# EthanD11/RS-VIO

Hardware: AMD Instinct MI355X
Metric: stereo frames/sec (tracker+BA) on 752×480 EuRoC stream; BA ms/iter at window=10 (higher is better)
Workload: dtype f32 (tracker) / f64 (BA)

## Files before the change

### rs-vio_amd/csrc/ba.hip

```cpp
#include <rccl/rccl.h>

#include <algorithm>
#include <chrono>
#include <cmath>
#include <cstdlib>
#include <cstring>
#include <string>
#include <sys/resource.h>
#include <numeric>
#include <stdexcept>
#include <vector>

#include "common.hpp"

#include "obs_pass.hpp"
#include "se3.hpp"
#include "wave.hpp"

#pragma clang fp contract(fast)

namespace rsvio {

namespace {

// ... 297 lines not shown
    const int i = blockIdx.x * blockDim.x + threadIdx.x;
    if (i < 7 * G.n_kf) {
        Wk.pose[0][i] = Wk.pose_init[i];
        Wk.pose[1][i] = Wk.pose_init[i];
    }
    if (i < 3 * G.n_lm) {
        Wk.pw[0][i] = Wk.pw_init[i];
        Wk.pw[1][i] = Wk.pw_init[i];
    }
    if (i == 0) {
        Wk.tick[1] = wall_clock64();
        *Wk.singular = 0;
        LmState s{};
        s.lambda = lambda0;
        s.nu = 2.0;
        *Wk.st = s;
    }
}

struct SlotLin {
    double V[6], gp[3], Wr[9], Ur[6], gr[3], cost;
};

__device__ __forceinline__ void slot_linearize(const Geometry& G, const Pose& P, const double p[3], int nobs,
                                               int cams, const double2 (&uvq)[2], bool fr, SlotLin& L) {
#pragma unroll
    for (int i = 0; i < 6; ++i) L.V[i] = 0.0;
#pragma unroll
    for (int i = 0; i < 3; ++i) L.gp[i] = 0.0;
#pragma unroll
    for (int i = 0; i < 9; ++i) L.Wr[i] = 0.0;
#pragma unroll
    for (int i = 0; i < 6; ++i) L.Ur[i] = 0.0;
#pragma unroll
    for (int i = 0; i < 3; ++i) L.gr[i] = 0.0;
    L.cost = 0.0;
#pragma unroll
    for (int o = 0; o < 2; ++o) {
        if (o >= nobs) break;
        double r[2], J[2][9];
        const double uv[2] = {uvq[o].x, uvq[o].y};
        linearize(p, P, G.TCB[(cams >> o) & 1].m, uv, r, J, true);
        double sq = r[0] * r[0] + r[1] * r[1], rho, wt;
        huber(sq, G.huber_delta, &rho, &wt);
        L.cost += 0.5 * rho;
        const double wr0 = wt * r[0], wr1 = wt * r[1];
        int k = 0;
#pragma unroll
        for (int a = 0; a < 3; ++a) {
#pragma unroll
            for (int c = a; c < 3; ++c) L.V[k++] += wt * (J[0][a] * J[0][c] + J[1][a] * J[1][c]);
            L.gp[a] += J[0][a] * wr0 + J[1][a] * wr1;
        }
        if (fr) {
            int u = 0;
#pragma unroll
            for (int a = 0; a < 3; ++a) {
#pragma unroll
                for (int c = 0; c < 3; ++c) L.Wr[a * 3 + c] += wt * (J[0][6 + a] * J[0][c] + J[1][6 + a] * J[1][c]);
#pragma unroll
                for (int c = a; c < 3; ++c) L.Ur[u++] += wt * (J[0][6 + a] * J[0][6 + c] + J[1][6 + a] * J[1][6 + c]);
                L.gr[a] += J[0][6 + a] * wr0 + J[1][6 + a] * wr1;
            }
        }
    }
}

__device__ __forceinline__ void wave_sync() {
// ... 2305 lines not shown
        if (i < n) {
            Wk.dc[i] = x[q];
            dcs[i] = x[q];
        }
    }
    __builtin_amdgcn_s_waitcnt(0xc07f);
    __builtin_amdgcn_wave_barrier();
    if (lane < G.n_kf) {
        double* qd = Wk.pose[1 - st->cur] + 7 * lane;
        if (fidx < 0) {
#pragma unroll
            for (int i = 0; i < 7; ++i) qd[i] = p7[i];
        } else {
            double qv[7];
            se3_plus(p7, dcs + 6 * fidx, qv);
#pragma unroll
            for (int i = 0; i < 7; ++i) qd[i] = qv[i];
        }
    }
    if (lane == 0) k5_result(st, 1, d2, gd);
    STAMP(5);
}

template <bool FUSED>
__device__ void k6_body(const Geometry& G, const Prob& Pr, const Work& Wk, int w, int lane, double (*sh)[64],
                        double (*shp)[64], double (*shs)[64], const P2P* PP = nullptr,
                        unsigned long long gen = 0, unsigned long long* k6tag = nullptr,
                        unsigned long long* k6part = nullptr) {
    const int s = 64 * w + lane;
    const int4 h0 = Pr.slot_hdr[2 * s], h1 = Pr.slot_hdr[2 * s + 1];
    const double2 uvq[2] = {Pr.slot_uv[2 * s], Pr.slot_uv[2 * s + 1]};
    const LmState* st = Wk.st;
    const bool act = h1.y > 0;
    const int kf = h0.x, l = h0.y, first = act ? h0.z : lane, nk = act ? h0.w : 1;
    const bool fr = h1.x >= 0;
    const int kfc = act ? kf : 0, lc = act ? l : 0, fc = (act && fr) ? h1.x : 0;
    double recb[2][18], Lmb[2][10], pcb[2][3], p7b[2][7], d6[6];
#pragma unroll
    for (int b = 0; b < 2; ++b) {
        const double2* wr = reinterpret_cast<const double2*>(Wk.raws[b] + (size_t)s * kRawF);
#pragma unroll
        for (int i = 0; i < 9; ++i) {
            const double2 x = wr[i];
            recb[b][2 * i] = x.x; recb[b][2 * i + 1] = x.y;
        }
        const double2* lr = reinterpret_cast<const double2*>(Wk.rawl[b] + (size_t)lc * kLmF);
#pragma unroll
        for (int i = 0; i < 5; ++i) {
            const double2 x = lr[i];
            Lmb[b][2 * i] = x.x; Lmb[b][2 * i + 1] = x.y;
        }
#pragma unroll
        for (int i = 0; i < 3; ++i) pcb[b][i] = Wk.pw[b][3 * lc + i];
#pragma unroll
        for (int i = 0; i < 7; ++i) p7b[b][i] = Wk.pose[b][7 * kfc + i];
    }
#pragma unroll
    for (int i = 0; i < 6; ++i) d6[i] = Wk.dc[6 * fc + i];
    const int done = st->done, solve_ok = st->solve_ok, cur = st->cur;
    const double lambda = st->lambda;
#pragma unroll
    for (int b = 0; b < 2; ++b) {
#pragma unroll
        for (int i = 0; i < 18; ++i) __asm__ volatile("" ::"v"(recb[b][i]));
#pragma unroll
        for (int i = 0; i < 10; ++i) __asm__ volatile("" ::"v"(Lmb[b][i]));
#pragma unroll
        for (int i = 0; i < 3; ++i) __asm__ volatile("" ::"v"(pcb[b][i]));
#pragma unroll
        for (int i = 0; i < 7; ++i) __asm__ volatile("" ::"v"(p7b[b][i]));
    }
    if (done || !solve_ok) return;
    STAMP(20);
    RTSTAMP(7);
    double Wv[18], Lm[10], pc[3], p7[7];
    {
        double rec[18];
#pragma unroll
        for (int i = 0; i < 18; ++i) rec[i] = cur ? recb[1][i] : recb[0][i];
        slot_w(rec, Wv);
#pragma unroll
        for (int i = 0; i < 10; ++i) Lm[i] = cur ? Lmb[1][i] : Lmb[0][i];
#pragma unroll
        for (int i = 0; i < 3; ++i) pc[i] = cur ? pcb[1][i] : pcb[0][i];
#pragma unroll
        for (int i = 0; i < 7; ++i) p7[i] = cur ? p7b[0][i] : p7b[1][i];
    }
    double t3[3] = {0.0, 0.0, 0.0};
    if (act && fr) {
#pragma unroll
        for (int c = 0; c < 3; ++c) {
            double acc = 0.0;
#pragma unroll
// ... 17 lines not shown
        double* pt = Wk.pw[1 - cur] + 3 * l;
        double dp2 = 0.0, gpdp = 0.0, p2 = 0.0;
#pragma unroll
        for (int c = 0; c < 3; ++c) {
            const double dp = (Vi[c][0] * rhs[0] + Vi[c][1] * rhs[1]) + Vi[c][2] * rhs[2];
            const double p = pc[c];
            const double q = p + dp;
            shp[c][lane] = q;
            pt[c] = q;
            dp2 += dp * dp;
            gpdp += Lm[LG + c] * dp;
            p2 += p * p;
        }
        shs[1][lane] = dp2;
        shs[2][lane] = gpdp;
        shs[3][lane] = p2;
    }
    if constexpr (FUSED) wave_sync(); else __syncthreads();
    STAMP(23);
    SlotLin L;
    if (act) {
        const Pose P = pose_from7(p7);
        const double q[3] = {shp[0][first], shp[1][first], shp[2][first]};
        slot_linearize(G, P, q, h1.y, h1.z, uvq, fr, L);
    } else {
        const Pose P{};
        const double q[3] = {0.0, 0.0, 1.0};
        slot_linearize(G, P, q, 0, 0, uvq, false, L);
    }
    shs[0][lane] = L.cost;
    if constexpr (FUSED) wave_sync(); else __syncthreads();
    STAMP(24);
    store_linearization<FUSED>(Wk, 1 - cur, s, lane, act, fr, first, nk, l, L, sh);
    STAMP(25);
    {
        double v[kPartD];
#pragma unroll
        for (int i = 0; i < kPartD; ++i) v[i] = wave_sum_det(shs[i][lane]);
        if (lane == 0)
#pragma unroll
            for (int i = 0; i < kPartD; ++i) Wk.partD[w * kPartD + i] = v[i];
        if (k6tag && lane < kPartD) {
            double vl = v[0];
#pragma unroll
            for (int i = 1; i < kPartD; ++i) vl = lane == i ? v[i] : vl;
            const unsigned long long b = (unsigned long long)__double_as_longlong(vl), t = gen << 32;
            const size_t nw = (size_t)G.n_wave;
            __hip_atomic_store(k6tag + (2 * lane) * nw + w, (b & 0xffffffffull) | t, __ATOMIC_RELAXED,
                               __HIP_MEMORY_SCOPE_AGENT);
            __hip_atomic_store(k6tag + (2 * lane + 1) * nw + w, (b >> 32) | t, __ATOMIC_RELAXED,
                               __HIP_MEMORY_SCOPE_AGENT);
        }
        if (k6part && lane < kPartD) {
            double vl = v[0];
#pragma unroll
            for (int i = 1; i < kPartD; ++i) vl = lane == i ? v[i] : vl;
            __hip_atomic_store(k6part + (size_t)w * kPartD + lane, (unsigned long long)__double_as_longlong(vl),
                               __ATOMIC_RELAXED, __HIP_MEMORY_SCOPE_AGENT);
        }
        if (PP && lane < PP->nranks) {
            const int par = (int)(gen & 1);
            double* q = p2p_tval(PP->peer[lane], par, PP->rank, w);
            q[0] = v[0]; q[1] = v[1]; q[2] = v[2]; q[3] = v[3];
            __threadfence_system();
            __hip_atomic_store(p2p_tflag(PP->peer[lane], par, PP->rank, w), gen, __ATOMIC_RELEASE,
                               __HIP_MEMORY_SCOPE_SYSTEM);
        }
    }
    STAMP(21);
    RTSTAMP(8);
}

__global__ __launch_bounds__(64) void ba_backsub_relinearize(Geometry G, Prob Pr, Work Wk) {
    __shared__ double sh[10][64];
    __shared__ double shp[3][64];
    __shared__ double shs[4][64];
    RTSTAMP(6);
    k6_body<false>(G, Pr, Wk, blockIdx.x, threadIdx.x, sh, shp, shs);
    RTSTAMP(9);
}

__global__ __launch_bounds__(64) void ba_backsub_relinearize_p2p(Geometry G, Prob Pr, Work Wk, P2P P,
                                                                 const unsigned long long* xgen) {
    __shared__ double sh[10][64];
    __shared__ double shp[3][64];
    __shared__ double shs[4][64];
    unsigned long long gen = *xgen;
    __asm__ volatile("" : "+s"(gen));
    k6_body<false>(G, Pr, Wk, blockIdx.x, threadIdx.x, sh, shp, shs, &P, gen);
}

template <int KU>
__device__ void k6_reduce_p2p(const Geometry& G, const Prob& Pr, const Work& Wk, const P2P& P,
                              unsigned long long* xgen, int* err, const unsigned long long* k6tag) {
    const int lane = threadIdx.x & 63;
    const LmState s = *Wk.st;
    const unsigned long long gen = *xgen + 1;
    if (s.done) return;
    const unsigned g32 = (unsigned)gen;
    const int nr = P.nranks, me = P.rank, par = (int)(gen & 1);
    const int el = 7 * G.n_kf - 1;
    double p0[3], p1[3];
// ... 200 lines not shown
    }
}

__global__ __launch_bounds__(64) void ba_reduce_trial(Geometry G, Prob Pr, Work Wk, int include_poses) {
    const LmState s = *Wk.st;
    if (s.done) return;
    double v[4];
    trial_scalars_wave(G, Pr, Wk, s, include_poses, v);
    if (threadIdx.x == 0)
        for (int k = 0; k < 4; ++k) Wk.trial4[k] = v[k];
}

constexpr int kK7Threads = 256;
#ifndef RSVIO_K7_BLOCKS
#define RSVIO_K7_BLOCKS 16
#endif
constexpr int kK7Blocks = RSVIO_K7_BLOCKS;
__device__ __forceinline__ void lm_decide_body(const Geometry& G, const Prob& Pr, const Work& Wk, int pre_reduced,
                                               const LmArgs& la, LmState* host, unsigned long long* htick,
                                               double* hout, const P2P* PP = nullptr,
                                               const unsigned long long* xgen = nullptr, int* err = nullptr) {
    STAMP(8);
    __shared__ LmState sd;
    if (threadIdx.x < 64) {
        const LmState d = lm_decide(G, Pr, Wk, Wk.st_prev, pre_reduced, la, PP, xgen, err);
        if (threadIdx.x == 0) {
            sd = d;
            if (blockIdx.x == 0) {
                LmState h = d;
                h.p2p_err = Wk.p2p_err ? *Wk.p2p_err : 0;
                *Wk.st = d;
                *host = h;
            }
        }
    }
    __syncthreads();
    const LmState s = sd;
    if (hout && s.done) {
        const double* pose = Wk.pose[s.cur];
        const double* pw = Wk.pw[s.cur];
        const int np = 7 * G.n_kf, n = np + 3 * G.n_lm;
        const int per = (((n + (int)gridDim.x - 1) / (int)gridDim.x) + 1) & ~1;
        const int i0 = (int)blockIdx.x * per, i1 = min(n, i0 + per);
        for (int i = i0 + 2 * (int)threadIdx.x; i < i1; i += 2 * kK7Threads) {
            const double a = i < np ? pose[i] : pw[i - np];
            if (i + 1 < i1) {
                const double b = i + 1 < np ? pose[i + 1] : pw[i + 1 - np];
                *reinterpret_cast<double2*>(hout + i) = make_double2(a, b);
            } else {
                hout[i] = a;
            }
        }
        __threadfence_system();
        __syncthreads();
        if (threadIdx.x == 0)
            __hip_atomic_store(htick + 4 + blockIdx.x, Wk.tick[1], __ATOMIC_RELEASE, __HIP_MEMORY_SCOPE_SYSTEM);
    }
    if (blockIdx.x == 0 && threadIdx.x == 0) {
        const unsigned long long t = Wk.tick[0] + 1;
        Wk.tick[0] = t;
        htick[1] = Wk.tick[1];
        htick[2] = wall_clock64();
        __threadfence_system();
        __hip_atomic_store(htick, t, __ATOMIC_RELEASE, __HIP_MEMORY_SCOPE_SYSTEM);
    }
    STAMP(10);
}

__global__ __launch_bounds__(kK7Threads) void ba_lm_decide(Geometry G, Prob Pr, Work Wk, int pre_reduced, LmArgs la,
                                                           LmState* host, unsigned long long* htick, double* hout) {
    lm_decide_body(G, Pr, Wk, pre_reduced, la, host, htick, hout);
}

__global__ __launch_bounds__(kK7Threads) void ba_lm_decide_p2p(Geometry G, Prob Pr, Work Wk, LmArgs la, LmState* host,
                                                               unsigned long long* htick, double* hout, P2P P,
                                                               const unsigned long long* xgen, int* err, int mode) {
    lm_decide_body(G, Pr, Wk, mode, la, host, htick, hout, &P, xgen, err);
}

// ... 46 lines not shown
template <int NF>
__global__ __launch_bounds__(64 * kBkWaves) void bab_camera_solve_blk(const WinDesc* __restrict__ D, int wi) {
    const WinDesc& d = D[blockIdx.x];
    const int skip = d.skip;
    const Prob Pr = d.Pr;
    const Work& Wk = d.W[wi];
    desc_touch(Pr.free_idx, Pr.dmap, Wk.pose[0], Wk.pose[1], Wk.cpart, Wk.partA, Wk.singular, Wk.st);
    if (skip) return;
    camera_solve_blk_body<NF>(d.G, Pr, Wk, 1);
}

__global__ __launch_bounds__(64) void bab_backsub_relinearize(const WinDesc* __restrict__ D, int wi) {
    const WinDesc& d = D[blockIdx.y];
    const int skip = d.skip, bound = d.G.n_wave;
    const Prob Pr = d.Pr;
    const Work& Wk = d.W[wi];
    desc_touch(Pr.slot_hdr, Pr.slot_uv, Wk.st, Wk.raws[0], Wk.raws[1], Wk.rawl[0], Wk.rawl[1], Wk.pw[0], Wk.pw[1],
               Wk.pose[0], Wk.pose[1], Wk.dc);
    if (skip | ((int)blockIdx.x >= bound)) return;
    __shared__ double sh[10][64];
    __shared__ double shp[3][64];
    __shared__ double shs[4][64];
    k6_body<false>(d.G, Pr, Wk, blockIdx.x, threadIdx.x, sh, shp, shs);
}

__global__ __launch_bounds__(kK7Threads) void bad_lm_decide(const WinDesc* __restrict__ D, int wi, LmArgs la,
                                                            LmState* host, unsigned long long* htick, double* hout) {
    const WinDesc& d = D[0];
    const Prob Pr = d.Pr;
    const Work& Wk = d.W[wi];
    lm_decide_body(d.G, Pr, Wk, 0, la, host, htick, hout);
}

__global__ __launch_bounds__(64) void bab_lm_decide(const WinDesc* __restrict__ D, int wi, LmArgs la, LmState* host) {
    const WinDesc& d = D[blockIdx.x];
    if (d.skip) return;
    const LmState s = lm_decide(d.G, d.Pr, d.W[wi], d.W[wi].st, 0, la);
    if (threadIdx.x == 0) {
        *d.W[wi].st = s;
        host[blockIdx.x] = s;
    }
}


__device__ void p2p_exchange(const double* msg, int n, const P2P& P, unsigned long long* xgen, int* err, double* out,
                             unsigned long long gen_pre = 0) {
// ... 238 lines not shown
        const bool topo = sl.exec && k_ok && same_cfg(sl.cfg, cfg) && sl.exp == export_on && sl.nf == G.n_free &&
                          sl.coll == coll;
        const bool hit = topo && (dm ? (sl.dptr == dptr() && sl.chunk == G.n_chunk && G.n_wave <= sl.wcap &&
                                        2 * G.n_wave > sl.wcap)
                                     : !sl.stale);
        if (hit) k = sl.k;
        if (!hit) {
            const auto tg0 = std::chrono::steady_clock::now();
            bool try_update = topo && sl.k == k && graph_update;
            if (try_update && hipEventQuery(sl.ev_launch) != hipSuccess) {
                (void)hipGetLastError();
                try_update = false;
            }
            if (!try_update) drop_slot(sl);
            if (hipStreamBeginCapture(stream, hipStreamCaptureModeThreadLocal) != hipSuccess) {
                (void)hipGetLastError();
                graphs_ok = false;
                return false;
            }
            bool ok = true;
            try {
                if (dm) {
                    enqueue_start_d(cfg.lambda_init, wcap);
                    for (int i = 0; i < k; ++i) enqueue_iteration_d(cfg, i, wcap);
                    enqueue_decide_d(cfg, k);
                } else {
                    enqueue_start(cfg.lambda_init);
                    for (int i = 0; i < k; ++i) enqueue_iteration(cfg, i);
                    enqueue_decide(cfg, k);
                }
            } catch (...) {
                ok = false;
            }
            hipGraph_t g = nullptr;
            if (hipStreamEndCapture(stream, &g) != hipSuccess) ok = false;
            const auto tg1 = std::chrono::steady_clock::now();
            bool updated = false;
            if (ok && try_update) {
                hipGraphNode_t err_node = nullptr;
                hipGraphExecUpdateResult r = hipGraphExecUpdateError;
                updated = hipGraphExecUpdate(sl.exec, g, &err_node, &r) == hipSuccess && r == hipGraphExecUpdateSuccess;
                if (!updated) {
                    (void)hipGetLastError();
                    drop_slot(sl);
                }
            }
            if (ok && !updated && hipGraphInstantiate(&sl.exec, g, nullptr, nullptr, 0) != hipSuccess) {
                sl.exec = nullptr;
                ok = false;
            }
            const auto tg2 = std::chrono::steady_clock::now();
// ... 25 lines not shown
        return true;
    }
    int last_iterations = 3;
    DevBuf<double> d_pose2, d_pw2;
    DevBuf<uint8_t> d_arena;
    HostBuf<uint8_t> h_arena;
    bool up_pending = false;
    struct ArenaLayout {
        size_t desc, pose_init, pw_init, free_idx, pb_fa, pb_fb, dmap, mask, lm_base, wave_fill, wave_lm, key, ouv, upload;
        size_t hdr, uv, pairs, total;
    } lay{};
    bool prof_env = false;
    bool prof_slow = false;
    std::string prof_maps;
    bool uv_env = true;
    bool early_env = false;
    bool stage_kernel = true;
    bool stage_split = true;
    const void* h_arena_dev = nullptr;
    HostBuf<double> h_out;
    bool state_export = false, export_on = false;
    bool state_fresh = false;
    std::vector<int> hs_free, hs_pb_fa, hs_pb_fb;
    DevBuf<double> d_raws, d_rawl, d_partA, d_partD, d_cpart, d_sys, d_dc, d_trial4;
    DevBuf<int> d_singular;
    size_t n_pad = 0;
    DevBuf<LmState> d_state;
    HostBuf<LmState> h_state;
    DevBuf<unsigned long long> d_tick;
    unsigned long long* h_tick = nullptr;
    unsigned long long n_tick = 0;
    bool settled = true, tick_wait = true;
    double wclk_khz = 1.0e5;
    ncclComm_t comm = nullptr;
    int nranks = 1, rank = 0;
    int coll = 0;
    bool sharded() const { return coll != 0; }
    double* xbuf = nullptr;
    P2P p2p{};
    bool p2p_opened[kP2PMax] = {};
    DevBuf<int> d_p2p_err;
    DevBuf<unsigned long long> d_xgen;
    DevBuf<int> d_xnw;
    DevBuf<unsigned long long> d_k6tag;
    DevBuf<unsigned> d_k6cnt;

    void init(const rsvio_ba_params& p) {
        P = p;
        if (P.max_keyframes < 2 || P.max_keyframes > kMaxFree + 1 || P.max_landmarks < 1 ||
            P.max_landmarks > (1 << 26) || P.max_observations < 1)
            throw std::invalid_argument("invalid BA capacities (max_keyframes in [2, 21], max_landmarks <= 2^26)");
        RSVIO_HIP(hipSetDevice(P.device));
        RSVIO_HIP(hipStreamCreateWithFlags(&stream, hipStreamNonBlocking));
        RSVIO_HIP(hipEventCreate(&ev0));
        RSVIO_HIP(hipEventCreate(&ev1));
        RSVIO_HIP(hipEventCreateWithFlags(&gv.ev_launch, hipEventDisableTiming));
        RSVIO_HIP(hipEventCreateWithFlags(&gd.ev_launch, hipEventDisableTiming));
        RSVIO_HIP(hipEventCreateWithFlags(&ev_desc, hipEventDisableTiming));
        const char* fv = std::getenv("RSVIO_P2P_FOLD");
        if (fv && fv[0] >= '0' && fv[0] <= '4') fold_lvl = fold_req = fv[0] - '0';
        const char* dv = std::getenv("RSVIO_BA_DESC");
        desc_on = !(dv && dv[0] == '0');
        const char* gu = std::getenv("RSVIO_BA_GRAPH_UPDATE");
        graph_update = !(gu && gu[0] == '0');
        h_state.alloc(1, hipHostMallocCoherent);
        h_out.alloc((size_t)7 * P.max_keyframes + (size_t)3 * P.max_landmarks, hipHostMallocCoherent);
        d_tick.alloc(2);
        RSVIO_HIP(hipMemset(d_tick.p, 0, 2 * sizeof(unsigned long long)));
        RSVIO_HIP(hipHostMalloc(reinterpret_cast<void**>(&h_tick), (4 + kK7Blocks) * sizeof(unsigned long long),
                                hipHostMallocCoherent));
        std::memset(h_tick, 0, (4 + kK7Blocks) * sizeof(unsigned long long));
        {
            int khz = 0;
            if (hipDeviceGetAttribute(&khz, hipDeviceAttributeWallClockRate, P.device) == hipSuccess && khz > 0)
                wclk_khz = khz;
        }
        const char* wv = std::getenv("RSVIO_BA_WAIT");
        tick_wait = !(wv && std::strcmp(wv, "sync") == 0);
        const char* ge = std::getenv("RSVIO_BA_GRAPHS");
        graphs_ok = !(ge && ge[0] == '0');
        const char* pv = std::getenv("RSVIO_BA_PROFILE");
        prof_env = pv != nullptr;
        prof_slow = pv && std::strcmp(pv, "slow") == 0;
        const char* u32v = std::getenv("RSVIO_BA_UV32");
        uv_env = !(u32v && u32v[0] == '0');
        const char* ecv = std::getenv("RSVIO_BA_EARLY_COPY");
        early_env = ecv && ecv[0] == '1';
        const char* stv = std::getenv("RSVIO_BA_STAGE");
        stage_kernel = !(stv && std::strcmp(stv, "sdma") == 0);
        if (stage_kernel) early_env = false;
        const char* ssv = std::getenv("RSVIO_BA_STAGE_SPLIT");
// ... 100 lines not shown
        int ntm = 0;
        auto faults = [] {
            struct rusage ru;
            getrusage(RUSAGE_THREAD, &ru);
            return (long)ru.ru_minflt;
        };
        long f0 = prof ? faults() : 0;
        auto mark = [&] {
            if (!prof) return;
            const auto t = std::chrono::steady_clock::now();
            const long f = faults();
            tms[ntm] = std::chrono::duration<double, std::micro>(t - tp0).count();
            flt[ntm++] = f - f0;
            tp0 = t;
            f0 = f;
        };
        if (pend.active) throw CallOrderError("set_problem: a solve is in flight (call rsvio_ba_wait first)");
        if (graph_update && gv.exec)
            gv.stale = true;
        else
            drop_slot(gv);
        solves_of_problem = 0;
        state_export = false;
        if (n_kf < 1 || n_kf > P.max_keyframes || n_lm < 0 || n_lm > P.max_landmarks || n_obs < 0 ||
            n_obs > P.max_observations)
            throw std::invalid_argument("problem exceeds the handle's capacities");
        auto& free_idx = hs_free;
        free_idx.assign(n_kf, -1);
        int n_free = 0;
        for (int k = 0; k < n_kf; ++k)
            if (!kf_fixed[k]) free_idx[k] = n_free++;
        if (n_free > kMaxFree) throw std::invalid_argument("too many free keyframes");
        if (n_free < 1) throw std::invalid_argument("no free keyframe");
        auto &pb_fa = hs_pb_fa, &pb_fb = hs_pb_fb;
        pb_fa.clear();
        pb_fb.clear();
        for (int a = 0; a < n_free; ++a)
            for (int b = a; b < n_free; ++b) {
                pb_fa.push_back(a);
                pb_fb.push_back(b);
            }
        const int n_pb = (int)pb_fa.size();
        const int n_chunk = kGrp * n_pb;
        auto al = [](size_t b) { return (b + 255) & ~(size_t)255; };
        const size_t nl1 = (size_t)std::max(n_lm, 1);
        ArenaLayout L{};
        size_t off = 0;
        L.desc = off;      off += al(sizeof(WinDesc));
        L.pose_init = off; off += al(sizeof(double) * 7 * (size_t)n_kf);
        L.pw_init = off;   off += al(sizeof(double) * 3 * nl1);
        L.free_idx = off;  off += al(sizeof(int) * (size_t)n_kf);
        L.pb_fa = off;     off += al(sizeof(int) * (size_t)n_pb);
        L.pb_fb = off;     off += al(sizeof(int) * (size_t)n_pb);
        L.dmap = off;      off += al(sizeof(int) * ((size_t)36 * n_pb + 12 * n_free));
        L.lm_base = off;   off += al(sizeof(int) * nl1);
        L.wave_fill = off; off += al(sizeof(int) * nl1);
        L.wave_lm = off;   off += al(sizeof(int) * (nl1 + 1));
        L.mask = off;      off += al(sizeof(unsigned long long) * nl1);
        L.key = off;       off += al(sizeof(unsigned) * std::max(n_obs, 1));
        L.ouv = off;       off += al(sizeof(double2) * std::max(n_obs, 1));
        L.upload = off;
        mark();
        if (up_pending) settle();
        if (h_arena.n < L.upload) {
            h_arena.alloc(L.upload + L.upload / 4, hipHostMallocCoherent);
            void* dp = nullptr;
            RSVIO_HIP(hipHostGetDevicePointer(&dp, h_arena.p, 0));
            h_arena_dev = dp;
        }
        uint8_t* hb = h_arena.p;
        mark();
        auto* m2 = reinterpret_cast<unsigned long long*>(hb + L.mask);
        auto* key = reinterpret_cast<unsigned*>(hb + L.key);
        bool uv32 = false;
        if (!observation_pass(n_obs, obs_lm, obs_kf, obs_cam, obs_uv, n_lm, n_kf, key, m2,
                              uv_env ? reinterpret_cast<float*>(hb + L.ouv) : nullptr, &uv32)) {
            std::memset(m2, 0, sizeof(unsigned long long) * (size_t)n_lm);
            int cl = -1;
            unsigned long long cm = 0;
            for (int i = 0; i < n_obs; ++i) {
                const int l = obs_lm[i], k = obs_kf[i], c = obs_cam[i];
                if (l < 0 || l >= n_lm || k < 0 || k >= n_kf || c > 1)
                    throw std::invalid_argument("observation index out of range");
                if (l != cl) {
                    if (cl >= 0) m2[cl] = cm;
                    cl = l;
                    cm = m2[l];
                }
// ... 61 lines not shown
        if (n_wave) wave_fill[n_wave - 1] = fill;
        wave_lm[n_wave] = n_lm;
        int stride = 1;
        for (int x = 0; x < kGrp; ++x) stride = std::max(stride, gl[x]);
        n_pad = (size_t)64 * n_wave;
        if (coll == 2 && fold_lvl == 2 && n_wave > kP2PWaves)
            throw std::invalid_argument("shard exceeds the folded P2P trial exchange (16384 waves): RSVIO_P2P_FOLD=1");
        mark();
        L.hdr = off;   off += al(sizeof(int4) * 2 * std::max<size_t>(n_pad, 1));
        L.uv = off;    off += al(sizeof(double2) * 2 * std::max<size_t>(n_pad, 1));
        L.pairs = off; off += al(sizeof(int4) * (size_t)n_chunk * stride);
        L.total = off;
        if (d_arena.n < L.total) {
            d_arena.alloc(L.total + L.total / 4);
            if (stage_split) stage(L.mask, L.upload);
            if (early_env)
                RSVIO_HIP(hipMemcpyAsync(d_arena.p + L.mask, hb + L.mask, L.upload - L.mask, hipMemcpyHostToDevice,
                                         stream));
        }
        lay = L;
        std::memcpy(hb + L.pose_init, pose7, sizeof(double) * 7 * (size_t)n_kf);
        if (n_lm) std::memcpy(hb + L.pw_init, pW, sizeof(double) * 3 * (size_t)n_lm);
        std::memcpy(hb + L.free_idx, free_idx.data(), sizeof(int) * (size_t)n_kf);
        std::memcpy(hb + L.pb_fa, pb_fa.data(), sizeof(int) * (size_t)n_pb);
        std::memcpy(hb + L.pb_fb, pb_fb.data(), sizeof(int) * (size_t)n_pb);
        if (n_free <= 10)
            mf_dense_map(n_free, n_pb, pb_fa.data(), pb_fb.data(), reinterpret_cast<int*>(hb + L.dmap));
        else
            mf_dense_map(n_free, n_pb, pb_fa.data(), pb_fb.data(), reinterpret_cast<int*>(hb + L.dmap),
                         6 * bk_template_nf(n_free), kBkLd);
        G.n_kf = n_kf; G.n_free = n_free; G.n_lm = n_lm; G.n_obs = n_obs; G.n_slot = (int)n_pad;
        G.n_pb = n_pb; G.n_wave = n_wave; G.n_chunk = n_chunk; G.pair_stride = stride;
        for (int k = 0, run = -1; k < kMaxFree; ++k) {
            run = std::max(run, cand[k]);
            G.env[k] = (unsigned char)(k >= n_free ? k : want_env ? std::max(k, run) : n_free - 1);
        }
        G.env_on = want_env ? 1 : 0;
        for (int c = 0; c < 2; ++c)
            for (int i = 0; i < 16; ++i) G.TCB[c].m[i] = TCB2[16 * c + i];
        grow_buffers();
        fill_desc(hdesc);
        std::memcpy(hb + L.desc, &hdesc, sizeof(WinDesc));
        mark();
        if (stage_kernel) {
            stage(0, stage_split ? L.mask : L.upload);
        } else {
            RSVIO_HIP(hipMemcpyAsync(d_arena.p, hb, early_env ? L.mask : L.upload, hipMemcpyHostToDevice, stream));
        }
        up_pending = true;
        {
            SlotSrc S;
            S.mask = reinterpret_cast<const unsigned long long*>(d_arena.p + L.mask);
            S.lm_base = reinterpret_cast<const int*>(d_arena.p + L.lm_base);
// ... 132 lines not shown
                if (k5_variant == 2) {
                    const dim3 b3(64 * kBkWaves);
                    switch (bk_template_nf(G.n_free)) {
                        case 13: hipLaunchKernelGGL(ba_camera_solve_blk<13>, g, b3, 0, stream, G, pr, wk, combine); break;
                        case 16: hipLaunchKernelGGL(ba_camera_solve_blk<16>, g, b3, 0, stream, G, pr, wk, combine); break;
                        default: hipLaunchKernelGGL(ba_camera_solve_blk<20>, g, b3, 0, stream, G, pr, wk, combine); break;
                    }
                    break;
                }
                const dim3 b2(64 * kX2Waves);
                if (G.n_free <= 13) hipLaunchKernelGGL(ba_camera_solve_x2<13>, g, b2, 0, stream, G, pr, wk, combine);
                else if (G.n_free <= 16) hipLaunchKernelGGL(ba_camera_solve_x2<16>, g, b2, 0, stream, G, pr, wk, combine);
                else hipLaunchKernelGGL(ba_camera_solve_x2<20>, g, b2, 0, stream, G, pr, wk, combine);
                break;
            }
        }
        RSVIO_HIP(hipGetLastError());
    }

    static LmArgs lm_args(const rsvio_lm_cfg& cfg) {
        return LmArgs{cfg.max_iterations, cfg.cost_tolerance, cfg.parameter_tolerance};
    }

    void enqueue_iteration(const rsvio_lm_cfg& cfg, int it) {
        const Prob pr = prob();
        const Work wk = work(it);
        if (p2p_fold()) {
            if (p2p_fold2() || p2p_fold4())
                hipLaunchKernelGGL(ba_schur_chunks_p2p, dim3(G.n_chunk), dim3(kSchurThreads), 0, stream, G, pr, wk,
                                   lm_args(cfg), p2p, d_xgen.p, d_p2p_err.p, p2p_fold4() ? 4 : 2);
            else
                hipLaunchKernelGGL(ba_schur_chunks, dim3(G.n_chunk), dim3(kSchurThreads), 0, stream, G, pr, wk,
                                   lm_args(cfg), 1);
            RSVIO_HIP(hipGetLastError());
            switch (G.n_free) {
#define RSVIO_CAMP(NF) \
    case NF:                                                                                                            \
        if (p2p.ll)                                                                                                     \
            hipLaunchKernelGGL((ba_camera_solve_mfma_p2p<NF, true>), dim3(1), dim3(kK5Threads), 0, stream, G, pr, wk,  \
                               p2p, d_xgen.p, d_p2p_err.p);                                                            \
        else                                                                                                            \
            hipLaunchKernelGGL((ba_camera_solve_mfma_p2p<NF, false>), dim3(1), dim3(kK5Threads), 0, stream, G, pr, wk, \
                               p2p, d_xgen.p, d_p2p_err.p);                                                            \
        break;
                RSVIO_CAMP(1) RSVIO_CAMP(2) RSVIO_CAMP(3) RSVIO_CAMP(4) RSVIO_CAMP(5)
                RSVIO_CAMP(6) RSVIO_CAMP(7) RSVIO_CAMP(8) RSVIO_CAMP(9) RSVIO_CAMP(10)
#undef RSVIO_CAMP
// ... 3 lines not shown
        } else {
            enqueue_linear_system(it, lm_args(cfg), false);
            launch_camera_solve(pr, wk, sharded() ? 0 : 1);
        }
        if (p2p_fold2()) {
            if (G.n_wave)
                hipLaunchKernelGGL(ba_backsub_relinearize_p2p, dim3(G.n_wave), dim3(64), 0, stream, G, pr, wk, p2p,
                                   d_xgen.p);
            RSVIO_HIP(hipGetLastError());
            return;
        }
        if (p2p_fold4()) {
            hipLaunchKernelGGL(ba_backsub_relinearize_p2p4, dim3(std::max(G.n_wave, 1)), dim3(64), 0, stream, G, pr,
                               wk, p2p, d_xgen.p, d_k6cnt.p, d_k6tag.p);
            RSVIO_HIP(hipGetLastError());
            return;
        }
        if (p2p_fold3()) {
            hipLaunchKernelGGL(ba_backsub_relinearize_p2p3, dim3(G.n_wave + 1), dim3(64), 0, stream, G, pr, wk, p2p,
                               d_xgen.p, d_p2p_err.p, d_k6tag.p);
            RSVIO_HIP(hipGetLastError());
            return;
        }
        if (G.n_wave) hipLaunchKernelGGL(ba_backsub_relinearize, dim3(G.n_wave), dim3(64), 0, stream, G, pr, wk);
        RSVIO_HIP(hipGetLastError());
        if (coll == 2) {
            hipLaunchKernelGGL(ba_p2p_trial, dim3(1), dim3(256), 0, stream, G, pr, wk, p2p, d_xgen.p, d_p2p_err.p);
            RSVIO_HIP(hipGetLastError());
        } else if (sharded()) {
            hipLaunchKernelGGL(ba_reduce_trial, dim3(1), dim3(64), 0, stream, G, pr, wk, rank == 0 ? 1 : 0);
            RSVIO_HIP(hipGetLastError());
            allreduce(d_trial4.p, 4);
        }
    }

    void enqueue_decide(const rsvio_lm_cfg& cfg, int it) {
        if (p2p_fold2() || p2p_fold4()) {
            hipLaunchKernelGGL(ba_lm_decide_p2p, dim3(export_on ? kK7Blocks : 1), dim3(kK7Threads), 0, stream, G,
                               prob(), work(it), lm_args(cfg), h_state.p, h_tick, export_on ? h_out.p : nullptr, p2p,
                               d_xgen.p, d_p2p_err.p, p2p_fold4() ? 4 : 2);
            RSVIO_HIP(hipGetLastError());
            return;
        }
        hipLaunchKernelGGL(ba_lm_decide, dim3(export_on ? kK7Blocks : 1), dim3(kK7Threads), 0, stream, G, prob(),
                           work(it), sharded() ? 1 : 0, lm_args(cfg), h_state.p, h_tick, export_on ? h_out.p : nullptr);
        RSVIO_HIP(hipGetLastError());
    }

    void enqueue_start_d(double lambda0, int wcap) {
        hipLaunchKernelGGL(bab_linearize, dim3(wcap, 1), dim3(64), 0, stream, dptr(), lambda0);
        RSVIO_HIP(hipGetLastError());
    }
    void enqueue_iteration_d(const rsvio_lm_cfg& cfg, int it, int wcap) {
        const int wi = it & 1;
        hipLaunchKernelGGL(bab_schur_chunks, dim3(G.n_chunk, 1), dim3(kSchurThreads), 0, stream, dptr(), wi, lm_args(cfg));
        RSVIO_HIP(hipGetLastError());
        switch (G.n_free) {
#define RSVIO_CAMD(NF) \
    case NF: hipLaunchKernelGGL(bab_camera_solve<NF>, dim3(1), dim3(kK5Threads), 0, stream, dptr(), wi); break;
            RSVIO_CAMD(1) RSVIO_CAMD(2) RSVIO_CAMD(3) RSVIO_CAMD(4) RSVIO_CAMD(5)
            RSVIO_CAMD(6) RSVIO_CAMD(7) RSVIO_CAMD(8) RSVIO_CAMD(9) RSVIO_CAMD(10)
#undef RSVIO_CAMD
            default: throw std::logic_error("descriptor mode: more than 10 free keyframes");
        }
        RSVIO_HIP(hipGetLastError());
        hipLaunchKernelGGL(bab_backsub_relinearize, dim3(wcap, 1), dim3(64), 0, stream, dptr(), wi);
        RSVIO_HIP(hipGetLastError());
    }
    void enqueue_decide_d(const rsvio_lm_cfg& cfg, int it) {
        hipLaunchKernelGGL(bad_lm_decide, dim3(export_on ? kK7Blocks : 1), dim3(kK7Threads), 0, stream, dptr(), it & 1,
                           lm_args(cfg), h_state.p, h_tick, export_on ? h_out.p : nullptr);
        RSVIO_HIP(hipGetLastError());
    }

    struct Pending {
        bool active = false, skipped = false;
        bool by_tick = false;
        rsvio_lm_cfg cfg{};
        int enq = 0, max_it = 0;
    } pend;

    void enqueue_chunk(int k) {
        settled = false;
        for (int i = 0; i < k; ++i) enqueue_iteration(pend.cfg, pend.enq + i);
        pend.enq += k;
        enqueue_decide(pend.cfg, pend.enq);
        ++n_tick;
        if (!pend.by_tick) RSVIO_HIP(hipEventRecord(ev1, stream));
    }

    void resync_ticks() noexcept {
        (void)hipStreamSynchronize(stream);
        (void)hipGetLastError();
        settled = true;
        unsigned long long t = 0;
        if (hipMemcpy(&t, d_tick.p, sizeof t, hipMemcpyDeviceToHost) == hipSuccess) n_tick = t;
        pend.active = false;
    }

    void start(const rsvio_lm_cfg& cfg) {
        if (!has_problem) throw std::invalid_argument("no problem uploaded");
        if (pend.active) throw CallOrderError("a solve is already in flight (call finish first)");
        try {
            start_impl(cfg);
        } catch (...) {
            resync_ticks();
            throw;
        }
    }

    void start_impl(const rsvio_lm_cfg& cfg) {
        G.huber_delta = cfg.huber_delta;
        G.chol = cfg.linear_solver == RSVIO_SOLVER_CHOLESKY ? 1 : 0;
        pend = Pending{};
        pend.active = true;
        pend.cfg = cfg;
        pend.by_tick = by_tick();
        state_export = false;
        if (!sharded() && (G.n_obs < 6 || G.n_obs < G.n_kf + G.n_lm)) {
            pend.skipped = true;
            return;
        }
        pend.max_it = std::max(cfg.max_iterations, 1);
        settled = false;
        state_fresh = false;
        if (!pend.by_tick) RSVIO_HIP(hipEventRecord(ev0, stream));
        int k = std::min(std::max(last_iterations, 1), pend.max_it);
        if (start_graph(cfg, k)) {
            ++n_tick;
            pend.enq += k;
            if (!pend.by_tick) RSVIO_HIP(hipEventRecord(ev1, stream));
        } else {
            enqueue_start(cfg.lambda_init);
            enqueue_chunk(k);
        }
    }

    void finish(rsvio_ba_result* res) {
        if (!pend.active) throw CallOrderError("no solve in flight");
        try {
            finish_impl(res);
        } catch (...) {
            resync_ticks();
            throw;
        }
    }

    void finish_impl(rsvio_ba_result* res) {
        pend.active = false;
        res->iterations = 0;
        if (pend.skipped) {
            res->status = RSVIO_LM_SKIPPED;
            res->initial_cost = res->final_cost = 0.0;
// ... 712 lines not shown
```

Baseline: 4892.

## Fuse final-iteration state export into cost-only backsub kernel and cache host tables

On the last iteration of a chunk, a new backsub kernel variant computes only the trial cost, skipping Jacobian and linearization stores. It also writes the current pose and landmark state into the host output buffer and stamps tick slots so lm_decide can skip its own export copy. If more iterations are then needed, the full relinearization is re-enqueued before the next chunk. Separately, the upload path skips rebuilding the pair and dense-map tables when a key of arena base, offsets, keyframe count and fixed mask is unchanged, which adds cache-validity risk.

```diff
diff --git a/rs-vio_amd/csrc/ba.hip b/rs-vio_amd/csrc/ba.hip
--- a/rs-vio_amd/csrc/ba.hip
+++ b/rs-vio_amd/csrc/ba.hip
@@ -343,28 +343,32 @@
     double V[6], gp[3], Wr[9], Ur[6], gr[3], cost;
 };
 
+template <bool COST_ONLY = false>
 __device__ __forceinline__ void slot_linearize(const Geometry& G, const Pose& P, const double p[3], int nobs,
                                                int cams, const double2 (&uvq)[2], bool fr, SlotLin& L) {
-#pragma unroll
-    for (int i = 0; i < 6; ++i) L.V[i] = 0.0;
-#pragma unroll
-    for (int i = 0; i < 3; ++i) L.gp[i] = 0.0;
-#pragma unroll
-    for (int i = 0; i < 9; ++i) L.Wr[i] = 0.0;
-#pragma unroll
-    for (int i = 0; i < 6; ++i) L.Ur[i] = 0.0;
-#pragma unroll
-    for (int i = 0; i < 3; ++i) L.gr[i] = 0.0;
+    if constexpr (!COST_ONLY) {
+#pragma unroll
+        for (int i = 0; i < 6; ++i) L.V[i] = 0.0;
+#pragma unroll
+        for (int i = 0; i < 3; ++i) L.gp[i] = 0.0;
+#pragma unroll
+        for (int i = 0; i < 9; ++i) L.Wr[i] = 0.0;
+#pragma unroll
+        for (int i = 0; i < 6; ++i) L.Ur[i] = 0.0;
+#pragma unroll
+        for (int i = 0; i < 3; ++i) L.gr[i] = 0.0;
+    }
     L.cost = 0.0;
 #pragma unroll
     for (int o = 0; o < 2; ++o) {
         if (o >= nobs) break;
         double r[2], J[2][9];
         const double uv[2] = {uvq[o].x, uvq[o].y};
-        linearize(p, P, G.TCB[(cams >> o) & 1].m, uv, r, J, true);
+        linearize(p, P, G.TCB[(cams >> o) & 1].m, uv, r, J, !COST_ONLY);
         double sq = r[0] * r[0] + r[1] * r[1], rho, wt;
         huber(sq, G.huber_delta, &rho, &wt);
         L.cost += 0.5 * rho;
+        if constexpr (COST_ONLY) continue;
         const double wr0 = wt * r[0], wr1 = wt * r[1];
         int k = 0;
 #pragma unroll
@@ -2716,11 +2720,21 @@
     STAMP(5);
 }
 
-template <bool FUSED>
+#ifndef RSVIO_EXPORT_FENCE
+#define RSVIO_EXPORT_FENCE 0
+#endif
+__device__ __forceinline__ void export_done() {
+#if RSVIO_EXPORT_FENCE
+    __builtin_amdgcn_fence(__ATOMIC_RELEASE, "");
+#else
+    __builtin_amdgcn_s_waitcnt(kWaitStores);
+#endif
+}
+template <bool FUSED, bool LAST = false>
 __device__ void k6_body(const Geometry& G, const Prob& Pr, const Work& Wk, int w, int lane, double (*sh)[64],
                         double (*shp)[64], double (*shs)[64], const P2P* PP = nullptr,
                         unsigned long long gen = 0, unsigned long long* k6tag = nullptr,
-                        unsigned long long* k6part = nullptr) {
+                        unsigned long long* k6part = nullptr, double* hout = nullptr) {
     const int s = 64 * w + lane;
     const int4 h0 = Pr.slot_hdr[2 * s], h1 = Pr.slot_hdr[2 * s + 1];
     const double2 uvq[2] = {Pr.slot_uv[2 * s], Pr.slot_uv[2 * s + 1]};
@@ -2751,6 +2765,18 @@
     }
 #pragma unroll
     for (int i = 0; i < 6; ++i) d6[i] = Wk.dc[6 * fc + i];
+    const int xnp = 7 * G.n_kf, xn = xnp + 3 * G.n_lm;
+    const int xi = (int)min(2ll * s, (long long)xn);
+    double xv[2][2] = {{0.0, 0.0}, {0.0, 0.0}};
+    unsigned long long xstamp = 0;
+    if constexpr (LAST) {
+#pragma unroll
+        for (int b = 0; b < 2; ++b)
+#pragma unroll
+            for (int e = 0; e < 2; ++e)
+                if (xi + e < xn) xv[b][e] = xi + e < xnp ? Wk.pose[b][xi + e] : Wk.pw[b][xi + e - xnp];
+        xstamp = Wk.tick[1];
+    }
     const int done = st->done, solve_ok = st->solve_ok, cur = st->cur;
     const double lambda = st->lambda;
 #pragma unroll
@@ -2763,6 +2789,34 @@
         for (int i = 0; i < 3; ++i) __asm__ volatile("" ::"v"(pcb[b][i]));
 #pragma unroll
         for (int i = 0; i < 7; ++i) __asm__ volatile("" ::"v"(p7b[b][i]));
+    }
+    if constexpr (LAST) {
+#pragma unroll
+        for (int e = 0; e < 2; ++e) __asm__ volatile("" ::"v"(xv[0][e]), "v"(xv[1][e]));
+        if (xi < xn) {
+            const double a = cur ? xv[1][0] : xv[0][0];
+            if (xi + 1 < xn)
+                *reinterpret_cast<double2*>(hout + xi) = make_double2(a, cur ? xv[1][1] : xv[0][1]);
+            else
+                hout[xi] = a;
+        }
+        const double* xpose = Wk.pose[cur];
+        const double* xpw = Wk.pw[cur];
+        for (long long i = xi + 128ll * G.n_wave; i < xn; i += 128ll * G.n_wave) {
+            const double a = i < xnp ? xpose[i] : xpw[i - xnp];
+            if (i + 1 < xn)
+                *reinterpret_cast<double2*>(hout + i) = make_double2(a, i + 1 < xnp ? xpose[i + 1] : xpw[i + 1 - xnp]);
+            else
+                hout[i] = a;
+        }
+        if (s == 0) {
+            Wk.tick[2] = xstamp;
+            Wk.tick[3] = (unsigned long long)(cur + 1);
+        }
+        if (done || !solve_ok) {
+            export_done();
+            return;
+        }
     }
     if (done || !solve_ok) return;
     STAMP(20);
@@ -2826,16 +2880,18 @@
     if (act) {
         const Pose P = pose_from7(p7);
         const double q[3] = {shp[0][first], shp[1][first], shp[2][first]};
-        slot_linearize(G, P, q, h1.y, h1.z, uvq, fr, L);
+        slot_linearize<LAST>(G, P, q, h1.y, h1.z, uvq, fr, L);
     } else {
         const Pose P{};
         const double q[3] = {0.0, 0.0, 1.0};
-        slot_linearize(G, P, q, 0, 0, uvq, false, L);
+        slot_linearize<LAST>(G, P, q, 0, 0, uvq, false, L);
     }
     shs[0][lane] = L.cost;
-    if constexpr (FUSED) wave_sync(); else __syncthreads();
-    STAMP(24);
-    store_linearization<FUSED>(Wk, 1 - cur, s, lane, act, fr, first, nk, l, L, sh);
+    if constexpr (!LAST) {
+        if constexpr (FUSED) wave_sync(); else __syncthreads();
+        STAMP(24);
+        store_linearization<FUSED>(Wk, 1 - cur, s, lane, act, fr, first, nk, l, L, sh);
+    }
     STAMP(25);
     {
         double v[kPartD];
@@ -2871,6 +2927,7 @@
                                __HIP_MEMORY_SCOPE_SYSTEM);
         }
     }
+    if constexpr (LAST) export_done();
     STAMP(21);
     RTSTAMP(8);
 }
@@ -2882,6 +2939,13 @@
     RTSTAMP(6);
     k6_body<false>(G, Pr, Wk, blockIdx.x, threadIdx.x, sh, shp, shs);
     RTSTAMP(9);
+}
+
+__global__ __launch_bounds__(64) void ba_backsub_trial_export(Geometry G, Prob Pr, Work Wk, double* hout) {
+    __shared__ double sh[10][64];
+    __shared__ double shp[3][64];
+    __shared__ double shs[4][64];
+    k6_body<false, true>(G, Pr, Wk, blockIdx.x, threadIdx.x, sh, shp, shs, nullptr, 0, nullptr, nullptr, hout);
 }
 
 __global__ __launch_bounds__(64) void ba_backsub_relinearize_p2p(Geometry G, Prob Pr, Work Wk, P2P P,
@@ -3128,6 +3192,13 @@
                                                const unsigned long long* xgen = nullptr, int* err = nullptr) {
     STAMP(8);
     __shared__ LmState sd;
+    unsigned long long xstamp = 0, xcur = 0, stamp = 0;
+    if (hout) {
+        stamp = Wk.tick[1];
+        xstamp = Wk.tick[2];
+        xcur = Wk.tick[3];
+        __asm__ volatile("" ::"v"(stamp), "v"(xstamp), "v"(xcur));
+    }
     if (threadIdx.x < 64) {
         const LmState d = lm_decide(G, Pr, Wk, Wk.st_prev, pre_reduced, la, PP, xgen, err);
         if (threadIdx.x == 0) {
@@ -3143,24 +3214,27 @@
     __syncthreads();
     const LmState s = sd;
     if (hout && s.done) {
-        const double* pose = Wk.pose[s.cur];
-        const double* pw = Wk.pw[s.cur];
-        const int np = 7 * G.n_kf, n = np + 3 * G.n_lm;
-        const int per = (((n + (int)gridDim.x - 1) / (int)gridDim.x) + 1) & ~1;
-        const int i0 = (int)blockIdx.x * per, i1 = min(n, i0 + per);
-        for (int i = i0 + 2 * (int)threadIdx.x; i < i1; i += 2 * kK7Threads) {
-            const double a = i < np ? pose[i] : pw[i - np];
-            if (i + 1 < i1) {
-                const double b = i + 1 < np ? pose[i + 1] : pw[i + 1 - np];
-                *reinterpret_cast<double2*>(hout + i) = make_double2(a, b);
-            } else {
-                hout[i] = a;
-            }
-        }
-        __threadfence_system();
-        __syncthreads();
+        const bool exported = xstamp == stamp && xcur == (unsigned long long)(s.cur + 1);
+        if (!exported) {
+            const double* pose = Wk.pose[s.cur];
+            const double* pw = Wk.pw[s.cur];
+            const int np = 7 * G.n_kf, n = np + 3 * G.n_lm;
+            const int per = (((n + (int)gridDim.x - 1) / (int)gridDim.x) + 1) & ~1;
+            const int i0 = (int)blockIdx.x * per, i1 = min(n, i0 + per);
+            for (int i = i0 + 2 * (int)threadIdx.x; i < i1; i += 2 * kK7Threads) {
+                const double a = i < np ? pose[i] : pw[i - np];
+                if (i + 1 < i1) {
+                    const double b = i + 1 < np ? pose[i + 1] : pw[i + 1 - np];
+                    *reinterpret_cast<double2*>(hout + i) = make_double2(a, b);
+                } else {
+                    hout[i] = a;
+                }
+            }
+            __threadfence_system();
+            __syncthreads();
+        }
         if (threadIdx.x == 0)
-            __hip_atomic_store(htick + 4 + blockIdx.x, Wk.tick[1], __ATOMIC_RELEASE, __HIP_MEMORY_SCOPE_SYSTEM);
+            __hip_atomic_store(htick + 4 + blockIdx.x, stamp, __ATOMIC_RELEASE, __HIP_MEMORY_SCOPE_SYSTEM);
     }
     if (blockIdx.x == 0 && threadIdx.x == 0) {
         const unsigned long long t = Wk.tick[0] + 1;
@@ -3253,6 +3327,20 @@
     __shared__ double shp[3][64];
     __shared__ double shs[4][64];
     k6_body<false>(d.G, Pr, Wk, blockIdx.x, threadIdx.x, sh, shp, shs);
+}
+
+__global__ __launch_bounds__(64) void bab_backsub_trial_export(const WinDesc* __restrict__ D, int wi, double* hout) {
+    const WinDesc& d = D[blockIdx.y];
+    const int skip = d.skip, bound = d.G.n_wave;
+    const Prob Pr = d.Pr;
+    const Work& Wk = d.W[wi];
+    desc_touch(Pr.slot_hdr, Pr.slot_uv, Wk.st, Wk.raws[0], Wk.raws[1], Wk.rawl[0], Wk.rawl[1], Wk.pw[0], Wk.pw[1],
+               Wk.pose[0], Wk.pose[1], Wk.dc, Wk.tick);
+    if (skip | ((int)blockIdx.x >= bound)) return;
+    __shared__ double sh[10][64];
+    __shared__ double shp[3][64];
+    __shared__ double shs[4][64];
+    k6_body<false, true>(d.G, Pr, Wk, blockIdx.x, threadIdx.x, sh, shp, shs, nullptr, 0, nullptr, nullptr, hout);
 }
 
 __global__ __launch_bounds__(kK7Threads) void bad_lm_decide(const WinDesc* __restrict__ D, int wi, LmArgs la,
@@ -3537,11 +3625,11 @@
             try {
                 if (dm) {
                     enqueue_start_d(cfg.lambda_init, wcap);
-                    for (int i = 0; i < k; ++i) enqueue_iteration_d(cfg, i, wcap);
+                    for (int i = 0; i < k; ++i) enqueue_iteration_d(cfg, i, wcap, i == k - 1);
                     enqueue_decide_d(cfg, k);
                 } else {
                     enqueue_start(cfg.lambda_init);
-                    for (int i = 0; i < k; ++i) enqueue_iteration(cfg, i);
+                    for (int i = 0; i < k; ++i) enqueue_iteration(cfg, i, i == k - 1);
                     enqueue_decide(cfg, k);
                 }
             } catch (...) {
@@ -3613,6 +3701,16 @@
     bool state_export = false, export_on = false;
     bool state_fresh = false;
     std::vector<int> hs_free, hs_pb_fa, hs_pb_fb;
+    struct TablesKey {
+        const uint8_t* base = nullptr;
+        size_t pb_fa = 0, pb_fb = 0, dmap = 0;
+        int n_kf = -1;
+        unsigned fixed = 0;
+        bool operator==(const TablesKey& o) const {
+            return base == o.base && pb_fa == o.pb_fa && pb_fb == o.pb_fb && dmap == o.dmap && n_kf == o.n_kf &&
+                   fixed == o.fixed;
+        }
+    } tables_key;
     DevBuf<double> d_raws, d_rawl, d_partA, d_partD, d_cpart, d_sys, d_dc, d_trial4;
     DevBuf<int> d_singular;
     size_t n_pad = 0;
@@ -3656,8 +3754,8 @@
         graph_update = !(gu && gu[0] == '0');
         h_state.alloc(1, hipHostMallocCoherent);
         h_out.alloc((size_t)7 * P.max_keyframes + (size_t)3 * P.max_landmarks, hipHostMallocCoherent);
-        d_tick.alloc(2);
-        RSVIO_HIP(hipMemset(d_tick.p, 0, 2 * sizeof(unsigned long long)));
+        d_tick.alloc(4);
+        RSVIO_HIP(hipMemset(d_tick.p, 0, 4 * sizeof(unsigned long long)));
         RSVIO_HIP(hipHostMalloc(reinterpret_cast<void**>(&h_tick), (4 + kK7Blocks) * sizeof(unsigned long long),
                                 hipHostMallocCoherent));
         std::memset(h_tick, 0, (4 + kK7Blocks) * sizeof(unsigned long long));
@@ -3804,6 +3902,8 @@
             drop_slot(gv);
         solves_of_problem = 0;
         state_export = false;
+        TablesKey tables_prev = tables_key;
+        tables_key = TablesKey{};
         if (n_kf < 1 || n_kf > P.max_keyframes || n_lm < 0 || n_lm > P.max_landmarks || n_obs < 0 ||
             n_obs > P.max_observations)
             throw std::invalid_argument("problem exceeds the handle's capacities");
@@ -3846,6 +3946,7 @@
         if (up_pending) settle();
         if (h_arena.n < L.upload) {
             h_arena.alloc(L.upload + L.upload / 4, hipHostMallocCoherent);
+            tables_prev = TablesKey{};
             void* dp = nullptr;
             RSVIO_HIP(hipHostGetDevicePointer(&dp, h_arena.p, 0));
             h_arena_dev = dp;
@@ -3953,13 +4054,21 @@
         std::memcpy(hb + L.pose_init, pose7, sizeof(double) * 7 * (size_t)n_kf);
         if (n_lm) std::memcpy(hb + L.pw_init, pW, sizeof(double) * 3 * (size_t)n_lm);
         std::memcpy(hb + L.free_idx, free_idx.data(), sizeof(int) * (size_t)n_kf);
-        std::memcpy(hb + L.pb_fa, pb_fa.data(), sizeof(int) * (size_t)n_pb);
-        std::memcpy(hb + L.pb_fb, pb_fb.data(), sizeof(int) * (size_t)n_pb);
-        if (n_free <= 10)
-            mf_dense_map(n_free, n_pb, pb_fa.data(), pb_fb.data(), reinterpret_cast<int*>(hb + L.dmap));
-        else
-            mf_dense_map(n_free, n_pb, pb_fa.data(), pb_fb.data(), reinterpret_cast<int*>(hb + L.dmap),
-                         6 * bk_template_nf(n_free), kBkLd);
+        TablesKey tk;
+        tk.base = hb;
+        tk.pb_fa = L.pb_fa; tk.pb_fb = L.pb_fb; tk.dmap = L.dmap;
+        tk.n_kf = n_kf;
+        for (int k = 0; k < n_kf; ++k) tk.fixed |= kf_fixed[k] ? 1u << k : 0u;
+        if (!(tk == tables_prev)) {
+            std::memcpy(hb + L.pb_fa, pb_fa.data(), sizeof(int) * (size_t)n_pb);
+            std::memcpy(hb + L.pb_fb, pb_fb.data(), sizeof(int) * (size_t)n_pb);
+            if (n_free <= 10)
+                mf_dense_map(n_free, n_pb, pb_fa.data(), pb_fb.data(), reinterpret_cast<int*>(hb + L.dmap));
+            else
+                mf_dense_map(n_free, n_pb, pb_fa.data(), pb_fb.data(), reinterpret_cast<int*>(hb + L.dmap),
+                             6 * bk_template_nf(n_free), kBkLd);
+        }
+        tables_key = tk;
         G.n_kf = n_kf; G.n_free = n_free; G.n_lm = n_lm; G.n_obs = n_obs; G.n_slot = (int)n_pad;
         G.n_pb = n_pb; G.n_wave = n_wave; G.n_chunk = n_chunk; G.pair_stride = stride;
         for (int k = 0, run = -1; k < kMaxFree; ++k) {
@@ -4138,7 +4247,8 @@
         return LmArgs{cfg.max_iterations, cfg.cost_tolerance, cfg.parameter_tolerance};
     }
 
-    void enqueue_iteration(const rsvio_lm_cfg& cfg, int it) {
+    bool lean_last() const { return export_on && !sharded() && G.n_wave > 0; }
+    void enqueue_iteration(const rsvio_lm_cfg& cfg, int it, bool last = false) {
         const Prob pr = prob();
         const Work wk = work(it);
         if (p2p_fold()) {
@@ -4188,7 +4298,10 @@
             RSVIO_HIP(hipGetLastError());
             return;
         }
-        if (G.n_wave) hipLaunchKernelGGL(ba_backsub_relinearize, dim3(G.n_wave), dim3(64), 0, stream, G, pr, wk);
+        if (last && lean_last())
+            hipLaunchKernelGGL(ba_backsub_trial_export, dim3(G.n_wave), dim3(64), 0, stream, G, pr, wk, h_out.p);
+        else if (G.n_wave)
+            hipLaunchKernelGGL(ba_backsub_relinearize, dim3(G.n_wave), dim3(64), 0, stream, G, pr, wk);
         RSVIO_HIP(hipGetLastError());
         if (coll == 2) {
             hipLaunchKernelGGL(ba_p2p_trial, dim3(1), dim3(256), 0, stream, G, pr, wk, p2p, d_xgen.p, d_p2p_err.p);
@@ -4217,7 +4330,7 @@
         hipLaunchKernelGGL(bab_linearize, dim3(wcap, 1), dim3(64), 0, stream, dptr(), lambda0);
         RSVIO_HIP(hipGetLastError());
     }
-    void enqueue_iteration_d(const rsvio_lm_cfg& cfg, int it, int wcap) {
+    void enqueue_iteration_d(const rsvio_lm_cfg& cfg, int it, int wcap, bool last = false) {
         const int wi = it & 1;
         hipLaunchKernelGGL(bab_schur_chunks, dim3(G.n_chunk, 1), dim3(kSchurThreads), 0, stream, dptr(), wi, lm_args(cfg));
         RSVIO_HIP(hipGetLastError());
@@ -4230,7 +4343,10 @@
             default: throw std::logic_error("descriptor mode: more than 10 free keyframes");
         }
         RSVIO_HIP(hipGetLastError());
-        hipLaunchKernelGGL(bab_backsub_relinearize, dim3(wcap, 1), dim3(64), 0, stream, dptr(), wi);
+        if (last && lean_last())
+            hipLaunchKernelGGL(bab_backsub_trial_export, dim3(wcap, 1), dim3(64), 0, stream, dptr(), wi, h_out.p);
+        else
+            hipLaunchKernelGGL(bab_backsub_relinearize, dim3(wcap, 1), dim3(64), 0, stream, dptr(), wi);
         RSVIO_HIP(hipGetLastError());
     }
     void enqueue_decide_d(const rsvio_lm_cfg& cfg, int it) {
@@ -4244,11 +4360,18 @@
         bool by_tick = false;
         rsvio_lm_cfg cfg{};
         int enq = 0, max_it = 0;
+        bool lean = false;
     } pend;
 
     void enqueue_chunk(int k) {
         settled = false;
-        for (int i = 0; i < k; ++i) enqueue_iteration(pend.cfg, pend.enq + i);
+        if (pend.lean) {
+            hipLaunchKernelGGL(ba_backsub_relinearize, dim3(G.n_wave), dim3(64), 0, stream, G, prob(),
+                               work(pend.enq - 1));
+            RSVIO_HIP(hipGetLastError());
+        }
+        for (int i = 0; i < k; ++i) enqueue_iteration(pend.cfg, pend.enq + i, i == k - 1);
+        pend.lean = lean_last();
         pend.enq += k;
         enqueue_decide(pend.cfg, pend.enq);
         ++n_tick;
@@ -4295,6 +4418,7 @@
         if (start_graph(cfg, k)) {
             ++n_tick;
             pend.enq += k;
+            pend.lean = lean_last();
             if (!pend.by_tick) RSVIO_HIP(hipEventRecord(ev1, stream));
         } else {
             enqueue_start(cfg.lambda_init);
```

Result: faster. 5023, median of 6 (+2.7%).
